# ShuoyiHU/pyqed

Measured on AMD Instinct MI355X. Metric: density-matrix steps/sec (N=128 Lindblad) + 2DES grid-points/sec at 1/2/4/8 GPU, higher is better.
Workload: dtype c128; 1 GPU; lindblad_n128_rk4_fp64 (BASELINE.json configs[1]); N=128, n_c_ops=1, batch_per_gpu=256, global_batch=256, parallelism=replicas x1 (independent density matrices per rank, no collective)

## Files before the change

### pyqed_amd/csrc/cgemm_dma128.hpp

```cpp
#pragma once
#include "cgemm_block.hpp"

namespace qd {

constexpr int cg_herm_ctile(int w, int nj) {
  constexpr unsigned short cols[8] = {0x3210, 0x7654, 0x7610, 0x5432, 0x7432, 0x6510, 0x5410, 0x7632};
  return (cols[w] >> (nj * 4)) & 15;
}
constexpr unsigned cg_herm_mask(int w, bool below) {
  unsigned m = 0;
  for (int mi = 0; mi < 2; ++mi)
    for (int nj = 0; nj < 4; ++nj) {
      const int R = mi == 0 ? (w >> 1) : 7 - (w >> 1), C = cg_herm_ctile(w, nj);
      if (below ? R > C : R < C) m |= 1u << (mi * 4 + nj);
    }
  return m;
}

struct CgAcc3 : CgAcc<128> { d4 p3[8]; };

typedef const __attribute__((address_space(1))) void cg_gvoid;
typedef __attribute__((address_space(3))) void cg_lvoid;

__device__ __forceinline__ const char* cg_uniform(const void* p) {
  const unsigned long long v = reinterpret_cast<unsigned long long>(p);
  const unsigned lo = __builtin_amdgcn_readfirstlane((unsigned)v);
  const unsigned hi = __builtin_amdgcn_readfirstlane((unsigned)(v >> 32));
  return reinterpret_cast<const char*>(((unsigned long long)hi << 32) | lo);
}

constexpr int cg_dma_a_kslot(int lr, int k) { return k ^ lr; }
constexpr int cg_dma_a_slot(int r0, int lr, int k) { return (r0 + lr) * CG_KT + cg_dma_a_kslot(lr, k); }
constexpr bool cg_dma_a_slot_bijective() {
  bool seen[128 * CG_KT] = {};
  for (int row = 0; row < 128; ++row)
    for (int k = 0; k < CG_KT; ++k) {
      const int s = cg_dma_a_slot(row & ~15, row & 15, k);
      if (s < 0 || s >= 128 * CG_KT || seen[s]) return false;
      if (cg_dma_a_kslot(row & 15, cg_dma_a_kslot(row & 15, k)) != k) return false;
      seen[s] = true;
    }
  return true;
}
constexpr bool cg_dma_a_slot_conflict_free() {
  for (int r0 = 0; r0 < 128; r0 += 16)
    for (int k = 0; k < CG_KT; ++k) {
      unsigned cols = 0;
      for (int lr = 0; lr < 16; ++lr) {
        const int s = cg_dma_a_slot(r0, lr, k);
        for (int l2 = 0; l2 < lr; ++l2)
          if (cg_dma_a_slot(r0, l2, k) == s) return false;
        cols |= 1u << (s & 15);
      }
      if (cols != 0xffffu) return false;
    }
  return true;
}
static_assert(cg_dma_a_slot_bijective(), "A-tile image: slots");
static_assert(cg_dma_a_slot_conflict_free(), "A-tile image: fragment read groups");

constexpr int cg_dma_b_slot(int k, int col) { return k * 128 + col; }
constexpr int cg_dma_b_k(int e) { return e >> 7; }
constexpr int cg_dma_b_col(int e) { return e & 127; }
constexpr bool cg_dma_b_slot_bijective() {
  bool seen[128 * CG_KT] = {};
  for (int k = 0; k < CG_KT; ++k)
    for (int col = 0; col < 128; ++col) {
      const int s = cg_dma_b_slot(k, col);
      if (s < 0 || s >= 128 * CG_KT || seen[s]) return false;
      if (cg_dma_b_k(s) != k || cg_dma_b_col(s) != col) return false;
      seen[s] = true;
    }
  return true;
}
static_assert(cg_dma_b_slot_bijective(), "B-tile image: slots");

struct CgDmaStage {
  const CgSeg* segs;
  int tps, lda, ldb;
  unsigned offA, offB;
  int wbase;
  __device__ __forceinline__ CgDmaStage(const CgSeg* s, int tps_, int lda_, int ldb_) : segs(s), tps(tps_), lda(lda_), ldb(ldb_) {
    int tid = threadIdx.x;
    asm volatile("" : "+v"(tid));
    const int row = tid >> 4;
    offA = (unsigned)(row * lda + cg_dma_a_kslot(row & 15, tid & 15)) * (unsigned)sizeof(c128);
    offB = (unsigned)(cg_dma_b_k(tid) * ldb + cg_dma_b_col(tid)) * (unsigned)sizeof(c128);
    wbase = __builtin_amdgcn_readfirstlane(tid & ~63);
  }
  __device__ __forceinline__ void issue(int t, CgLds<128>& L, int buf) const {
    const CgSeg sg = segs[t / tps];
    issue_at(sg.A, sg.B, (t % tps) * CG_KT, L, buf);
  }
  __device__ __forceinline__ void issue_at(const c128* A, const c128* B, int kt, CgLds<128>& L, int buf) const {
    const char* ga = cg_uniform(A + kt);
    const char* gb = cg_uniform(B + (size_t)kt * ldb);
#pragma unroll
    for (int q = 0; q < 4; ++q) {
      __builtin_amdgcn_global_load_lds((cg_gvoid*)(ga + (size_t)q * 32 * lda * sizeof(c128) + offA),
                                       (cg_lvoid*)(&L.a[buf][wbase + CG_WG * q]), 16, 0, 0);
      __builtin_amdgcn_global_load_lds((cg_gvoid*)(gb + (size_t)q * 4 * ldb * sizeof(c128) + offB),
                                       (cg_lvoid*)(&L.b[buf][wbase + CG_WG * q]), 16, 0, 0);
    }
  }
  __device__ __forceinline__ void piece(const char* ga, const char* gb, int i, CgLds<128>& L, int buf) const {
    const int q = i & 3;
    if (i >= 4)
      __builtin_amdgcn_global_load_lds((cg_gvoid*)(gb + (size_t)q * 4 * ldb * sizeof(c128) + offB),
                                       (cg_lvoid*)(&L.b[buf][wbase + CG_WG * q]), 16, 0, 0);
    else
      __builtin_amdgcn_global_load_lds((cg_gvoid*)(ga + (size_t)q * 32 * lda * sizeof(c128) + offA),
                                       (cg_lvoid*)(&L.a[buf][wbase + CG_WG * q]), 16, 0, 0);
  }
  __device__ __forceinline__ void issue_b_at(const c128* B, int kt, CgLds<128>& L, int buf) const {
    const char* gb = cg_uniform(B + (size_t)kt * ldb);
#pragma unroll
    for (int q = 0; q < 4; ++q)
      __builtin_amdgcn_global_load_lds((cg_gvoid*)(gb + (size_t)q * 4 * ldb * sizeof(c128) + offB),
                                       (cg_lvoid*)(&L.b[buf][wbase + CG_WG * q]), 16, 0, 0);
  }
};

struct CgNoHook {
  __device__ __forceinline__ void operator()(int) const {}
};

constexpr int CG_STAGE_PER = 2;
struct CgDmaStageHook {
  const CgDmaStage& st;
  CgLds<128>& L;
  const char* ga;
  const char* gb;
  int buf;
  __device__ __forceinline__ void operator()(int p) const {
    static_assert(4 % CG_STAGE_PER == 0, "a point's pieces belong to one half");
    if (p * CG_STAGE_PER >= 8) return;
    if (p * CG_STAGE_PER < 4 ? !ga : !gb) return;
#pragma unroll
    for (int i = p * CG_STAGE_PER; i < (p + 1) * CG_STAGE_PER; ++i) st.piece(ga, gb, i, L, buf);
  }
};

#ifdef QD_PHASE_TIMING
#define CG_KSTAMP_PARAM , unsigned long long (&tk)[6], int tko
#define CG_KSTAMP_ARG(a, o) , a, o
#define CG_KSTAMP_TOP unsigned long long ks0_ = clock64(), ks1_ = ks0_;
#define CG_KSTAMP_END                  \
  cg_sched_fence();                    \
  const unsigned long long ks2_ = clock64(); \
  cg_sched_fence();
#define CG_KSTAMP_BAR                              \
  {                                                \
    const unsigned long long ks3_ = clock64();     \
    tk[tko] += ks1_ - ks0_;                        \
    tk[tko + 1] += ks2_ - ks1_;                    \
    tk[tko + 2] += ks3_ - ks2_;                    \
    ks0_ = ks3_;                                   \
  }
template <class H>
struct CgStampHook {
  const H& h;
  unsigned long long& at;
  __device__ __forceinline__ void operator()(int p) const {
    h(p);
    if (p == 0) {
      cg_sched_fence();
      at = clock64();
      cg_sched_fence();
    }
  }
};
#define CG_KSTAMP_HOOK(h) CgStampHook<decltype(h)>{h, ks1_}
#else
#define CG_KSTAMP_PARAM
#define CG_KSTAMP_ARG(a, o)
#define CG_KSTAMP_TOP
#define CG_KSTAMP_END
#define CG_KSTAMP_BAR
#define CG_KSTAMP_HOOK(h) h
#endif

template <unsigned SK, int Q0, int Q1, class Hook = CgNoHook>
__device__ __forceinline__ void cg_dma_ksteps(const CgLds<128>& L, int buf, CgAcc3& acc, const int (&r0)[2],
                                              const int (&c0)[4], const Hook& hook = Hook()) {
  constexpr int BT = 128, MW = 2, NW = 4;
  constexpr unsigned LIVE = 0xffu & ~SK;
  const int lane = threadIdx.x & 63;
  const int lr = lane & 15, lk = lane >> 4;
#pragma unroll
  for (int q = Q0; q < Q1; ++q) {
    const int kk = 4 * q;
    c128 a[MW];
    double sa[MW];
#pragma unroll
    for (int mi = 0; mi < MW; ++mi) {
      a[mi] = L.a[buf][cg_dma_a_slot(r0[mi], lr, kk + lk)];
      if ((LIVE >> (mi * 4)) & 15u) sa[mi] = a[mi].re + a[mi].im;
    }
#pragma unroll
    for (int h = 0; h < NW; h += 2) {
      c128 b[2];
      double sb[2];
#pragma unroll
      for (int j = 0; j < 2; ++j) {
        const int nj = h + j;
        if (((LIVE >> nj) | (LIVE >> (4 + nj))) & 1u) {
          b[j] = L.b[buf][cg_dma_b_slot(kk + lk, c0[nj] + lr)];
          sb[j] = b[j].re + b[j].im;
        }
      }
      hook(2 * q + h / 2);
#pragma unroll
      for (int mi = 0; mi < MW; ++mi)
#pragma unroll
        for (int j = 0; j < 2; ++j) {
          const int nj = h + j;
          if (SK & (1u << (mi * 4 + nj))) continue;
          acc.re[mi][nj] = __builtin_amdgcn_mfma_f64_16x16x4f64(a[mi].re, b[j].re, acc.re[mi][nj], 0, 0, 0);
        }
#pragma unroll
      for (int mi = 0; mi < MW; ++mi)
#pragma unroll
        for (int j = 0; j < 2; ++j) {
          const int nj = h + j;
          if (SK & (1u << (mi * 4 + nj))) continue;
          acc.im[mi][nj] = __builtin_amdgcn_mfma_f64_16x16x4f64(a[mi].im, b[j].im, acc.im[mi][nj], 0, 0, 0);
          acc.p3[mi * 4 + nj] = __builtin_amdgcn_mfma_f64_16x16x4f64(sa[mi], sb[j], acc.p3[mi * 4 + nj], 0, 0, 0);
        }
    }
  }
}

__device__ __forceinline__ void cg_dma_scale(CgAcc3& acc, unsigned M, double S) {
#pragma unroll
  for (int mi = 0; mi < 2; ++mi)
#pragma unroll
    for (int nj = 0; nj < 4; ++nj)
      if (M & (1u << (mi * 4 + nj))) {
        acc.re[mi][nj] *= S;
        acc.im[mi][nj] *= S;
        acc.p3[mi * 4 + nj] *= S;
      }
}

__device__ __forceinline__ void cg_dma_zero(CgAcc3& acc) {
#pragma unroll
  for (int mi = 0; mi < 2; ++mi)
#pragma unroll
    for (int nj = 0; nj < 4; ++nj) {
      acc.re[mi][nj] = d4{0.0, 0.0, 0.0, 0.0};
      acc.im[mi][nj] = d4{0.0, 0.0, 0.0, 0.0};
      acc.p3[mi * 4 + nj] = d4{0.0, 0.0, 0.0, 0.0};
    }
}

__device__ __forceinline__ void cg_dma_finalise(CgAcc3& acc) {
#pragma unroll
  for (int mi = 0; mi < 2; ++mi)
#pragma unroll
    for (int nj = 0; nj < 4; ++nj) {
      const d4 p1 = acc.re[mi][nj], p2 = acc.im[mi][nj];
      acc.re[mi][nj] = p1 - p2;
      acc.im[mi][nj] = (acc.p3[mi * 4 + nj] - p1) - p2;
      asm volatile("" : "+v"(acc.re[mi][nj]), "+v"(acc.im[mi][nj]));
    }
}

__device__ __forceinline__ void cg_dma_block_gemm_stream(const c128* A, const c128* B, const c128* nA, const c128* nB,
                                                         bool first, int K, int lda, int ldb, CgLds<128>& L,
                                                         CgAcc3& acc) {
  constexpr int MW = CgCfg<128>::MW, NW = CgCfg<128>::NW, WC = CgCfg<128>::WC, NQ = CG_KT / 4;
  const int wave = __builtin_amdgcn_readfirstlane(threadIdx.x >> 6);
  const int wr0 = (wave / WC) * (MW * 16), wc0 = (wave % WC) * (NW * 16);
  const int r0[2] = {wr0, wr0 + 16}, c0[4] = {wc0, wc0 + 16, wc0 + 32, wc0 + 48};
  cg_dma_zero(acc);
  const int T = K / CG_KT;
  const CgDmaStage st(nullptr, T, lda, ldb);
  if (first) {
    st.issue_at(A, B, 0, L, 0);
    __syncthreads();
  }
  for (int t = 0; t < T; ++t) {
    if (t + 1 < T) st.issue_at(A, B, (t + 1) * CG_KT, L, (t + 1) & 1);
    else st.issue_at(nA, nB, 0, L, 0);
    cg_sched_fence();
    cg_dma_ksteps<0u, 0, NQ>(L, t & 1, acc, r0, c0);
    __syncthreads();
  }
  cg_dma_finalise(acc);
}

template <int W, unsigned SK>
__device__ __forceinline__ void cg_dma_herm_x_range(int t0, int t1, int T, const CgDmaStage& st, CgLds<128>& L,
                                                    CgAcc3& acc) {
  constexpr int NQ = CG_KT / 4, R0 = 16 * (W >> 1), R1 = 16 * (7 - (W >> 1));
  const int r0[2] = {R0, R1};
  const int c0[4] = {16 * cg_herm_ctile(W, 0), 16 * cg_herm_ctile(W, 1), 16 * cg_herm_ctile(W, 2),
                     16 * cg_herm_ctile(W, 3)};
  for (int t = t0; t < t1; ++t) {
    if (t + 1 < T) st.issue(t + 1, L, (t + 1) & 1);
    cg_sched_fence();
    cg_dma_ksteps<SK, 0, NQ>(L, t & 1, acc, r0, c0);
    __syncthreads();
  }
}

__device__ __forceinline__ void cg_dma_herm_x_gemm(const CgSeg* segs, int nseg, int K, int lda, int ldb, CgLds<128>& L,
                                                   CgAcc3& acc, bool pre = false) {
  const int wave = __builtin_amdgcn_readfirstlane(threadIdx.x >> 6);
  cg_dma_zero(acc);
  const int tps = K / CG_KT, T = nseg * tps;
  const CgDmaStage st(segs, tps, lda, ldb);
  if (!pre) {
    st.issue(0, L, 0);
    __syncthreads();
  }
  auto run = [&](auto wc) {
    constexpr int W = decltype(wc)::value;
    cg_dma_herm_x_range<W, 0u>(0, tps, T, st, L, acc);
    cg_dma_scale(acc, cg_herm_mask(W, false), 0.5);
    cg_dma_herm_x_range<W, cg_herm_mask(W, true)>(tps, T, T, st, L, acc);
    cg_dma_scale(acc, cg_herm_mask(W, false), 2.0);
  };
#define QD_HT(w) \
  case w: run(std::integral_constant<int, w>{}); break;
  switch (wave) {
    QD_HT(0) QD_HT(1) QD_HT(2) QD_HT(3) QD_HT(4) QD_HT(5) QD_HT(6) default: QD_HT(7)
  }
#undef QD_HT
  cg_dma_finalise(acc);
}

template <unsigned M>
__device__ __forceinline__ void cg_dma_finalise_live(CgAcc3& acc) {
#pragma unroll
  for (int mi = 0; mi < 2; ++mi)
#pragma unroll
    for (int nj = 0; nj < 4; ++nj) {
      if (!(M & (1u << (mi * 4 + nj)))) continue;
      const d4 p1 = acc.re[mi][nj], p2 = acc.im[mi][nj];
      acc.re[mi][nj] = p1 - p2;
      acc.im[mi][nj] = (acc.p3[mi * 4 + nj] - p1) - p2;
      asm volatile("" : "+v"(acc.re[mi][nj]), "+v"(acc.im[mi][nj]));
    }
}


enum CgStart { CG_START_COLD, CG_START_TILE0, CG_START_TWO };
__device__ __forceinline__ void cg_dma_block_gemm_stream_h(const c128* A, const c128* B, const c128* nA, const c128* nB,
                                                           CgStart start, int K, int lda, int ldb, CgLds<128>& L,
                                                           CgAcc3& acc CG_KSTAMP_PARAM) {
  constexpr int MW = CgCfg<128>::MW, NW = CgCfg<128>::NW, WC = CgCfg<128>::WC, NQ = CG_KT / 4;
  const int wave = __builtin_amdgcn_readfirstlane(threadIdx.x >> 6);
  const int wr0 = (wave / WC) * (MW * 16), wc0 = (wave % WC) * (NW * 16);
  const int r0[2] = {wr0, wr0 + 16}, c0[4] = {wc0, wc0 + 16, wc0 + 32, wc0 + 48};
  cg_dma_zero(acc);
  const int T = K / CG_KT;
  const CgDmaStage st(nullptr, T, lda, ldb);
  if (start == CG_START_COLD) {
    st.issue_at(A, B, 0, L, 0);
    __syncthreads();
  }
  CG_KSTAMP_TOP
  for (int t = 0; t < T; ++t) {
    const bool more = t + 1 < T;
    const char* ga = more ? cg_uniform(A + (t + 1) * CG_KT) : nA ? cg_uniform(nA) : nullptr;
    const char* gb = cg_uniform(more ? B + (size_t)(t + 1) * CG_KT * ldb : nB);
    if (start == CG_START_TWO && t == 0) gb = nullptr;
    const CgDmaStageHook hook{st, L, ga, gb, more ? (t + 1) & 1 : 0};
    cg_sched_fence();
    cg_dma_ksteps<0u, 0, NQ>(L, t & 1, acc, r0, c0, CG_KSTAMP_HOOK(hook));
    CG_KSTAMP_END
    asm volatile("s_waitcnt vmcnt(0)" ::: "memory");
    __syncthreads();
    CG_KSTAMP_BAR
  }
  cg_dma_finalise(acc);
}

__device__ __forceinline__ void cg_dma_a_tile_write(const CgAcc3& acc, int mi, int nj, int row0 , int lane,
                                                    CgLds<128>& L, int buf) {
#pragma unroll
  for (int e = 0; e < 4; ++e)
    L.a[buf][cg_dma_a_slot(row0, (lane >> 4) + 4 * e, lane & 15)] = cmk(acc.re[mi][nj][e], acc.im[mi][nj][e]);
}

template <int W>
__device__ __forceinline__ void cg_dma_herm_d_gemm_h(const CgSeg* segs, const c128* nA, int nseg, int K, int lda,
                                                     int ldb, CgLds<128>& L, CgAcc3& acc, bool two CG_KSTAMP_PARAM) {
  constexpr unsigned SK = cg_herm_mask(W, true);
  constexpr int NQ = CG_KT / 4, R0 = 16 * (W >> 1), R1 = 16 * (7 - (W >> 1));
  const int r0[2] = {R0, R1};
  const int c0[4] = {16 * cg_herm_ctile(W, 0), 16 * cg_herm_ctile(W, 1), 16 * cg_herm_ctile(W, 2),
                     16 * cg_herm_ctile(W, 3)};
  cg_dma_zero(acc);
  const int tps = K / CG_KT, T = nseg * tps;
  const CgDmaStage st(segs, tps, lda, ldb);
  int t = 0;
  CG_KSTAMP_TOP
  if (two) {
    cg_sched_fence();
    const CgNoHook none;
    cg_dma_ksteps<SK, 0, NQ>(L, 0, acc, r0, c0, CG_KSTAMP_HOOK(none));
    CG_KSTAMP_END
    asm volatile("s_waitcnt vmcnt(0)" ::: "memory");
    __syncthreads();
    CG_KSTAMP_BAR
    t = 1;
  }
  for (; t < T; ++t) {
    const char *ga = nullptr, *gb = nullptr;
    if (t + 1 == T) {
      if (nA) ga = cg_uniform(nA);
    } else {
      const CgSeg sg = segs[(t + 1) / tps];
      const int kt = ((t + 1) % tps) * CG_KT;
      ga = cg_uniform(sg.A + kt);
      gb = cg_uniform(sg.B + (size_t)kt * ldb);
    }
    const CgDmaStageHook hook{st, L, ga, gb, (t + 1) & 1};
    cg_sched_fence();
    cg_dma_ksteps<SK, 0, NQ>(L, t & 1, acc, r0, c0, CG_KSTAMP_HOOK(hook));
    CG_KSTAMP_END
    asm volatile("s_waitcnt vmcnt(0)" ::: "memory");
    __syncthreads();
    CG_KSTAMP_BAR
  }
}

}
```

### pyqed_amd/csrc/glf_eig_jump.hip

```cpp
#include "glf_eig_jump_kernel.hpp"

#include <algorithm>

using namespace qd;

namespace {

__global__ void eig_jump_prep_kernel(const c128* W, const c128* Wi, const c128* Et, int ne, c128* Wdh, c128* Widh,
                                     c128* eT) {
  constexpr int Np = JUMP_NP;
  constexpr size_t NN = (size_t)Np * Np;
  for (size_t e = blockIdx.x * (size_t)blockDim.x + threadIdx.x; e < NN; e += (size_t)gridDim.x * blockDim.x) {
    const int i = (int)(e / Np), j = (int)(e % Np);
    const size_t t = (size_t)j * Np + i;
    Wdh[t] = cscale(cconj(W[e]), 0.5);
    Widh[t] = cscale(cconj(Wi[e]), 0.5);
    for (int m = 0; m < ne; ++m) eT[m * NN + t] = Et[m * NN + e];
  }
}

}

extern "C" int qd_lindblad_rk4_eig_jump(const qd_c128* mu, const qd_c128* At, const qd_c128* W, const qd_c128* Winv,
                                        qd_c128* rho, int B, int N, double dt, int nsteps, const qd_c128* Et, int ne,
                                        qd_c128* obs, void* stream) {
  QD_CHECK_ARG(mu && At && W && Winv && rho, "qd_lindblad_rk4_eig_jump: mu, At, W, Winv and rho must be non-null");
  QD_CHECK_ARG(N > 64 && N <= JUMP_NP, "qd_lindblad_rk4_eig_jump: N=%d outside (64, 128]", N);
  QD_CHECK_ARG(B >= 1 && nsteps >= 0 && ne >= 0, "qd_lindblad_rk4_eig_jump: bad sizes B=%d nsteps=%d ne=%d", B, nsteps,
               ne);
  QD_CHECK_ARG(ne == 0 || (Et && obs), "qd_lindblad_rk4_eig_jump: Et/obs null but ne=%d", ne);
  hipStream_t st = (hipStream_t)stream;
  WsScope wss_(st);
  constexpr int Np = JUMP_NP;
  constexpr size_t NN = (size_t)Np * Np;
  int rc;
  void* wops = nullptr;
  if ((rc = workspace(WS_LINDBLAD_OPS, (size_t)(2 + ne) * NN * sizeof(c128), &wops, st))) return rc;
  c128* Wdh = (c128*)wops;
  c128* Widh = Wdh + NN;
  c128* eT = Widh + NN;
  const bool pad = Np != N;
  const size_t per = 2 * NN;
  void* wst = nullptr;
  if ((rc = workspace(WS_LINDBLAD, ((size_t)B * per + (pad ? (size_t)B * NN : 0)) * sizeof(c128), &wst, st))) return rc;
  c128* scratch = (c128*)wst;
  c128* rho_p = pad ? scratch + (size_t)B * per : (c128*)rho;
  hipLaunchKernelGGL(eig_jump_prep_kernel, dim3((int)(NN / 256)), dim3(256), 0, st, (const c128*)W, (const c128*)Winv,
                     (const c128*)Et, ne, Wdh, Widh, eT);
  QD_HIP(hipGetLastError());
  if (pad && (rc = glf_pad((const c128*)rho, rho_p, B, N, Np, st))) return rc;
  LindbladJumpParams p{};
  p.At = (const c128*)At;
  p.W = (const c128*)W;
  p.Wi = (const c128*)Winv;
  p.Wdh = Wdh;
  p.Widh = Widh;
  p.mu = (const c128*)mu;
  p.eT = eT;
  p.rho = rho_p;
  p.ws = scratch;
  p.obs = (c128*)obs;
  p.ne = ne;
  p.nsteps = nsteps;
  p.dt = dt;
  p.tbuf = nullptr;
#ifdef QD_PHASE_TIMING
  QD_HIP(hipMalloc(&p.tbuf, (size_t)B * QD_TSTRIDE * sizeof(unsigned long long)));
  QD_HIP(hipMemsetAsync(p.tbuf, 0, (size_t)B * QD_TSTRIDE * sizeof(unsigned long long), st));
#endif
  note_path("glf_eig_jump");
  hipLaunchKernelGGL(lindblad_eig_jump_kernel, dim3(B), dim3(CG_WG), 0, st, p);
  QD_HIP(hipGetLastError());
  if (pad && (rc = glf_unpad(rho_p, (c128*)rho, B, N, Np, st))) return rc;
#ifdef QD_PHASE_TIMING
  {
    std::vector<unsigned long long> t((size_t)B * QD_TSTRIDE);
    QD_HIP(hipStreamSynchronize(st));
    QD_HIP(hipMemcpy(t.data(), p.tbuf, t.size() * sizeof(unsigned long long), hipMemcpyDeviceToHost));
    (void)hipFree(p.tbuf);
    int dev = 0, khz = 100000;
    (void)hipGetDevice(&dev);
    (void)hipDeviceGetAttribute(&khz, hipDeviceAttributeWallClockRate, dev);
    const char* names[6] = {"basis-changes", nullptr, "gemm", "update", "obs", "lds-pass"};
    std::fprintf(stderr, "[qd phase timing] eig_jump N=%d B=%d nsteps=%d, us per step (basis-changes: per call; mean "
                 "over workgroups):", N, B, nsteps);
    for (int q = 0; q < 6; ++q) {
      if (!names[q]) continue;
      double s = 0;
      for (int b = 0; b < B; ++b) s += (double)t[(size_t)b * QD_TSTRIDE + q];
      std::fprintf(stderr, " %s %.2f", names[q], s / B / (khz * 1e-3) / (q == 0 ? 1 : std::max(1, nsteps)));
    }
    double cyc = 0, wt = 0;
    for (int b = 0; b < B; ++b) {
      cyc += (double)t[(size_t)b * QD_TSTRIDE + QD_TCLK];
      wt += (double)t[(size_t)b * QD_TSTRIDE + QD_TWALL];
    }
    std::fprintf(stderr, " | shader clock %.0f MHz\n", wt > 0 ? cyc / (wt / (khz * 1e3)) / 1e6 : 0.0);
  }
#endif
  return QD_OK;
}
```

### pyqed_amd/csrc/glf_eig_jump_kernel.hpp

```cpp
#pragma once
#include "glf_herm_k.hpp"

namespace qd {

struct LindbladJumpParams {
  const c128* At;
  const c128* W;
  const c128* Wi;
  const c128* Wdh;
  const c128* Widh;
  const c128* mu;
  const c128* eT;
  c128* rho;
  c128* ws;
  c128* obs;
  int ne, nsteps;
  double dt;
  unsigned long long* tbuf;
};

namespace {

constexpr int JUMP_NP = 128;
constexpr int JUMP_NPRE = 3;

template <int W>
__device__ __forceinline__ void jump_r_loads(const c128* r, int Np, int lane, c128 (&rq)[8][4]) {
  const unsigned vu = (unsigned)((lane >> 4) * Np + (lane & 15)) * (unsigned)sizeof(c128);
#pragma unroll
  for (int mi = 0; mi < 2; ++mi)
#pragma unroll
    for (int nj = 0; nj < 4; ++nj) {
      const int R = mi == 0 ? (W >> 1) : 7 - (W >> 1), C = cg_herm_ctile(W, nj);
#pragma unroll
      for (int e = 0; e < 4; ++e) {
        const unsigned su = (unsigned)((16 * R + 4 * e) * Np) * (unsigned)sizeof(c128);
        rq[mi * 4 + nj][e] = *reinterpret_cast<const c128*>(reinterpret_cast<const char*>(r + 16 * C) + (vu + su));
      }
    }
}
template <int W>
__device__ __forceinline__ void jump_mu_reads(const c128* muS, int lane, c128 (&mj)[4], c128 (&mi_)[2][4]) {
#pragma unroll
  for (int nj = 0; nj < 4; ++nj) mj[nj] = muS[16 * cg_herm_ctile(W, nj) + (lane & 15)];
#pragma unroll
  for (int mi = 0; mi < 2; ++mi)
#pragma unroll
    for (int e = 0; e < 4; ++e) mi_[mi][e] = muS[16 * (mi == 0 ? (W >> 1) : 7 - (W >> 1)) + (lane >> 4) + 4 * e];
}
__device__ __forceinline__ void jump_init_mr(CgAcc3& acc, c128 (&rq)[8][4], const c128 (&mj)[4],
                                             const c128 (&mi_)[2][4]) {
#pragma unroll
  for (int mi = 0; mi < 2; ++mi)
#pragma unroll
    for (int nj = 0; nj < 4; ++nj) {
#pragma unroll
      for (int e = 0; e < 4; ++e) {
        const c128 a = mi_[mi][e], b = mj[nj], x = rq[mi * 4 + nj][e];
        const double mre = 0.5 * (a.re * b.re + a.im * b.im), mim = 0.5 * (a.im * b.re - a.re * b.im);
        rq[mi * 4 + nj][e] = cmk(mre * x.re - mim * x.im, mre * x.im + mim * x.re);
      }
#pragma unroll
      for (int e = 0; e < 4; ++e) asm volatile("" : "+v"(rq[mi * 4 + nj][e].re), "+v"(rq[mi * 4 + nj][e].im));
    }
  cg_sched_fence();
#pragma unroll
  for (int mi = 0; mi < 2; ++mi)
#pragma unroll
    for (int nj = 0; nj < 4; ++nj)
#pragma unroll
      for (int e = 0; e < 4; ++e) {
        const c128 t = rq[mi * 4 + nj][e];
        acc.re[mi][nj][e] = t.re;
        acc.im[mi][nj][e] = 0.0;
        acc.p3[mi * 4 + nj][e] = t.re + t.im;
      }
}

template <int W>
__device__ __forceinline__ void jump_gemm(const c128* A, const c128* B, const c128* r, bool mr, const c128* muS, int Np,
                                          int lane, CgLds<128>& L, CgAcc3& acc) {
  constexpr int NQ = CG_KT / 4, R0 = 16 * (W >> 1), R1 = 16 * (7 - (W >> 1));
  const int r0[2] = {R0, R1};
  const int c0[4] = {16 * cg_herm_ctile(W, 0), 16 * cg_herm_ctile(W, 1), 16 * cg_herm_ctile(W, 2),
                     16 * cg_herm_ctile(W, 3)};
  const int T = Np / CG_KT;
  const CgDmaStage st(nullptr, T, Np, Np);
  if (mr) {
    c128 rq[8][4], mj[4], mi_[2][4];
    jump_r_loads<W>(r, Np, lane, rq);
    jump_mu_reads<W>(muS, lane, mj, mi_);
    asm volatile("s_waitcnt lgkmcnt(0)" ::: "memory");
    cg_sched_fence();
    st.issue_at(A, B, 0, L, 0);
    cg_sched_fence();
    jump_init_mr(acc, rq, mj, mi_);
  } else {
    st.issue_at(A, B, 0, L, 0);
    cg_dma_zero(acc);
  }
  __syncthreads();
  for (int t = 0; t < T; ++t) {
    const bool more = t + 1 < T;
    const char* ga = more ? cg_uniform(A + (t + 1) * CG_KT) : nullptr;
    const char* gb = more ? cg_uniform(B + (size_t)(t + 1) * CG_KT * Np) : nullptr;
    const CgDmaStageHook hook{st, L, ga, gb, (t + 1) & 1};
    cg_sched_fence();
    cg_dma_ksteps<0u, 0, NQ>(L, t & 1, acc, r0, c0, hook);
    asm volatile("s_waitcnt vmcnt(0)" ::: "memory");
    __syncthreads();
  }
  cg_dma_finalise(acc);
}

template <int W, int NPRE>
__device__ __forceinline__ void jump_update(const CgAcc<128>& A, const c128* KL, int lane, c128 (&q)[8][4],
                                            const c128* base, c128* rn, int Np, double a, double hc) {
  const int lr = lane >> 4, lc = lane & 15;
  const unsigned vu = (unsigned)(lr * Np + lc) * (unsigned)sizeof(c128);
  const unsigned vm = (unsigned)(lc * Np + lr) * (unsigned)sizeof(c128);
  int n = 0;
#pragma unroll
  for (int mi = 0; mi < 2; ++mi)
#pragma unroll
    for (int nj = 0; nj < 4; ++nj) {
      const int R = mi == 0 ? (W >> 1) : 7 - (W >> 1), C = cg_herm_ctile(W, nj);
      if (R > C) continue;
      if (n >= 1) {
        cg_sched_fence();
        herm_k_rho_loads<W>(base, Np, lane, q, n - 1 + NPRE, n + NPRE);
        cg_sched_fence();
      }
      ++n;
      c128 m[4];
#pragma unroll
      for (int r = 0; r < 4; ++r) {
        const int ra = lr + 4 * r;
        if (R < C) m[r] = KL[HermKL::tile(R, C) + HermKL::slot(ra, lc)];
        else m[r] = KL[HermKL::DIAG0 + R * 128 + HermKL::dslot(ra, lc)];
      }
#pragma unroll
      for (int r = 0; r < 4; ++r) {
        const c128 x = cmk(A.re[mi][nj][r], A.im[mi][nj][r]);
        const int ra = lr + 4 * r;
        const c128 k = cadd(x, R == C && ra == lc ? cconj(x) : m[r]);
        c128 v = cadd(cscale(q[mi * 4 + nj][r], a), cscale(k, hc));
        if (R == C && ra == lc) v.im = 0.0;
        const unsigned su = (unsigned)((16 * R + 4 * r) * Np) * (unsigned)sizeof(c128);
        const unsigned sm = (unsigned)(16 * C * Np) * (unsigned)sizeof(c128);
        char* u = reinterpret_cast<char*>(rn + 16 * C) + (vu + su);
        char* t = reinterpret_cast<char*>(rn + 16 * R + 4 * r) + (vm + sm);
        if (R < C || ra <= lc) *reinterpret_cast<c128*>(u) = v;
        if (R < C || ra < lc) *reinterpret_cast<c128*>(t) = cconj(v);
      }
    }
}

template <int W>
__device__ __forceinline__ void jump_store_y(const CgAcc<128>& A, c128* Y, int Np, int lane) {
  const unsigned vu = (unsigned)((lane >> 4) * Np + (lane & 15)) * (unsigned)sizeof(c128);
#pragma unroll
  for (int mi = 0; mi < 2; ++mi)
#pragma unroll
    for (int nj = 0; nj < 4; ++nj) {
      const int R = mi == 0 ? (W >> 1) : 7 - (W >> 1), C = cg_herm_ctile(W, nj);
#pragma unroll
      for (int e = 0; e < 4; ++e) {
        const unsigned su = (unsigned)((16 * R + 4 * e) * Np) * (unsigned)sizeof(c128);
        *reinterpret_cast<c128*>(reinterpret_cast<char*>(Y + 16 * C) + (vu + su)) = cmk(A.re[mi][nj][e], A.im[mi][nj][e]);
      }
    }
}

__global__ __launch_bounds__(CG_WG) void lindblad_eig_jump_kernel(LindbladJumpParams p) {
  constexpr int BT = JUMP_NP;
  constexpr size_t NN = (size_t)JUMP_NP * JUMP_NP;
  int Np = JUMP_NP;
  asm volatile("" : "+s"(Np));
  __shared__ CgLds<BT> L;
  __shared__ c128 sred[CG_WG / 64];
  __shared__ c128 muS[JUMP_NP];

  const int b = blockIdx.x;
  c128* rho = p.rho + (size_t)b * NN;
  c128* ws = p.ws + (size_t)b * 2 * NN;
  c128* rbuf1 = ws + NN;
  c128* obs = p.obs ? p.obs + (size_t)b * (p.nsteps + 1) * p.ne : nullptr;
  if (threadIdx.x < JUMP_NP) muS[threadIdx.x] = p.mu[threadIdx.x];
  __syncthreads();

  CgAcc3 A;
  QD_TIMING_DECL
#ifdef QD_PHASE_TIMING
  unsigned long long txf = 0;
#endif

  const int nit = 4 * p.nsteps + 4;
  for (int it = 0; it < nit; ++it) {
    const bool xf = it < 2 || it >= nit - 2, ypass = it == 0 || it == nit - 2;
    const int stage = (it - 2) & 3;
    const c128* r = (xf || stage == 0) ? rho : ((stage - 1) & 1) ? rbuf1 : ws;
    c128* rn = (xf || stage == 3) ? rho : (stage & 1) ? rbuf1 : ws;
    const c128* oa = it == 0 ? p.Wi : it == nit - 2 ? p.W : xf ? ws : p.At;
    const c128* ob = it == 1 ? p.Widh : it == nit - 1 ? p.Wdh : r;
    double dts = p.dt;
    asm volatile("" : "+s"(dts));
    const double hc = wave_uniform(xf ? 1.0 : glf_horner_coef(dts, stage)), ab = wave_uniform(xf ? 0.0 : 1.0);
#ifdef QD_PHASE_TIMING
    unsigned long long tkeep[6] = {tacc[0], tacc[1], tacc[2], tacc[3], tacc[4], tacc[5]};
#endif
    {
      static_assert(HermKL::SIZE * sizeof(c128) <= sizeof(CgLds<BT>), "LDS k image");
      c128* KL = reinterpret_cast<c128*>(&L);
      const int wave = __builtin_amdgcn_readfirstlane(threadIdx.x >> 6);
      auto pass = [&](auto wc) {
        constexpr int W = decltype(wc)::value;
        {
          int tid = threadIdx.x;
          asm volatile("" : "+v"(tid));
          jump_gemm<W>(oa, ob, r, !xf, muS, Np, tid & 63, L, A);
        }
        QD_TMARK(2);
        int tid = threadIdx.x;
        asm volatile("" : "+v"(tid));
        const int lane = tid & 63;
        int Npe = Np;
        asm volatile("" : "+s"(Npe));
        if (ypass) {
          jump_store_y<W>(A, ws, Npe, lane);
          return;
        }
        c128 q[8][4];
        herm_k_publish<W>(A, KL, lane);
        cg_sched_fence();
        herm_k_rho_loads<W>(rho, Npe, lane, q, 0, JUMP_NPRE);
        __syncthreads();
        QD_TMARK(5);
        jump_update<W, JUMP_NPRE>(A, KL, lane, q, rho, rn, Npe, ab, hc);
      };
#define QD_JW(w) \
  case w: pass(std::integral_constant<int, w>{}); break;
      switch (wave) { QD_JW(0) QD_JW(1) QD_JW(2) QD_JW(3) QD_JW(4) QD_JW(5) QD_JW(6) default: QD_JW(7) }
#undef QD_JW
      __syncthreads();
    }
    QD_TMARK(3);
#ifdef QD_PHASE_TIMING
    if (xf)
      for (int q = 0; q < 6; ++q) {
        txf += tacc[q] - tkeep[q];
        tacc[q] = tkeep[q];
      }
#endif
    if (p.ne > 0 && (it == 1 || (!xf && stage == 3))) {
      wg_observables_batch(rho, p.eT, p.ne, NN, obs + (size_t)((it - 1) / 4) * p.ne, sred);
      QD_TMARK(4);
    }
  }
#ifdef QD_PHASE_TIMING
  tacc[0] += txf;
#endif
  QD_TIMING_FLUSH
}

}
}
```

Measured before the change: 988,700 density-matrix steps/s.

## Exploit Hermitian structure in jump-operator GEMM and fuse stage tail via LDS

```diff
diff --git a/pyqed_amd/csrc/cgemm_dma128.hpp b/pyqed_amd/csrc/cgemm_dma128.hpp
--- a/pyqed_amd/csrc/cgemm_dma128.hpp
+++ b/pyqed_amd/csrc/cgemm_dma128.hpp
@@ -428,4 +428,93 @@
   }
 }
 
-}
+constexpr unsigned cg_xh_row(unsigned m, int mi) { return (m >> (mi * 4)) & 15u; }
+constexpr unsigned cg_xh_col(unsigned m, int nj) { return ((m >> nj) | (m >> (4 + nj))) & 1u; }
+constexpr int cg_xh_diag_row(unsigned dg, int nj) { return (dg >> nj) & 1u ? 0 : (dg >> (4 + nj)) & 1u ? 1 : -1; }
+
+template <unsigned FS, unsigned SW, unsigned DG, int Q0, int Q1, class Hook = CgNoHook>
+__device__ __forceinline__ void cg_dma_ksteps_xh(const CgLds<128>& L, int buf, CgAcc3& acc, const int (&r0)[2],
+                                                 const int (&c0)[4], const Hook& hook = Hook()) {
+  static_assert((SW & ~FS) == 0u && (DG & ~FS) == 0u && (DG & SW) == 0u, "SW and DG are disjoint subsets of FS");
+  constexpr int MW = 2, NW = 4;
+  const int lane = threadIdx.x & 63;
+  const int lr = lane & 15, lk = lane >> 4;
+#pragma unroll
+  for (int q = Q0; q < Q1; ++q) {
+    const int kk = 4 * q;
+    c128 a[MW], br[MW];
+    double sa[MW], sbr[MW], dbr[MW];
+#pragma unroll
+    for (int mi = 0; mi < MW; ++mi) {
+      if (cg_xh_row(FS, mi)) {
+        a[mi] = L.a[buf][cg_dma_a_slot(r0[mi], lr, kk + lk)];
+        sa[mi] = a[mi].re + a[mi].im;
+      }
+      if (cg_xh_row(SW, mi)) {
+        br[mi] = L.b[buf][cg_dma_b_slot(kk + lk, r0[mi] + lr)];
+        dbr[mi] = br[mi].re - br[mi].im;
+        if (cg_xh_row(DG, mi)) sbr[mi] = br[mi].re + br[mi].im;
+      }
+    }
+#pragma unroll
+    for (int h = 0; h < NW; h += 2) {
+      c128 b[2], ac[2];
+      double sb[2], dac[2];
+#pragma unroll
+      for (int j = 0; j < 2; ++j) {
+        const int nj = h + j, dm = cg_xh_diag_row(DG, nj);
+        if (cg_xh_col(FS, nj)) {
+          if (dm >= 0 && cg_xh_row(SW, dm)) {
+            b[j] = br[dm];
+            sb[j] = sbr[dm];
+          } else {
+            b[j] = L.b[buf][cg_dma_b_slot(kk + lk, c0[nj] + lr)];
+            sb[j] = b[j].re + b[j].im;
+          }
+        }
+        if (cg_xh_col(SW, nj)) {
+          if (dm >= 0) ac[j] = a[dm];
+          else ac[j] = L.a[buf][cg_dma_a_slot(c0[nj], lr, kk + lk)];
+          dac[j] = ac[j].re - ac[j].im;
+        }
+      }
+      hook(2 * q + h / 2);
+#pragma unroll
+      for (int mi = 0; mi < MW; ++mi)
+#pragma unroll
+        for (int j = 0; j < 2; ++j) {
+          const int nj = h + j;
+          if (!(FS & (1u << (mi * 4 + nj)))) continue;
+          acc.re[mi][nj] = __builtin_amdgcn_mfma_f64_16x16x4f64(a[mi].re, b[j].re, acc.re[mi][nj], 0, 0, 0);
+        }
+#pragma unroll
+      for (int mi = 0; mi < MW; ++mi)
+#pragma unroll
+        for (int j = 0; j < 2; ++j) {
+          const int nj = h + j;
+          if (!(FS & (1u << (mi * 4 + nj)))) continue;
+          acc.im[mi][nj] = __builtin_amdgcn_mfma_f64_16x16x4f64(a[mi].im, b[j].im, acc.im[mi][nj], 0, 0, 0);
+          acc.p3[mi * 4 + nj] = __builtin_amdgcn_mfma_f64_16x16x4f64(sa[mi], sb[j], acc.p3[mi * 4 + nj], 0, 0, 0);
+        }
+#pragma unroll
+      for (int mi = 0; mi < MW; ++mi)
+#pragma unroll
+        for (int j = 0; j < 2; ++j) {
+          const int nj = h + j;
+          if (!(SW & (1u << (mi * 4 + nj)))) continue;
+          acc.re[mi][nj] = __builtin_amdgcn_mfma_f64_16x16x4f64(br[mi].re, ac[j].re, acc.re[mi][nj], 0, 0, 0);
+        }
+#pragma unroll
+      for (int mi = 0; mi < MW; ++mi)
+#pragma unroll
+        for (int j = 0; j < 2; ++j) {
+          const int nj = h + j;
+          if (!(SW & (1u << (mi * 4 + nj)))) continue;
+          acc.im[mi][nj] = __builtin_amdgcn_mfma_f64_16x16x4f64(br[mi].im, ac[j].im, acc.im[mi][nj], 0, 0, 0);
+          acc.p3[mi * 4 + nj] = __builtin_amdgcn_mfma_f64_16x16x4f64(dbr[mi], dac[j], acc.p3[mi * 4 + nj], 0, 0, 0);
+        }
+    }
+  }
+}
+
+}
diff --git a/pyqed_amd/csrc/glf_eig_jump.hip b/pyqed_amd/csrc/glf_eig_jump.hip
--- a/pyqed_amd/csrc/glf_eig_jump.hip
+++ b/pyqed_amd/csrc/glf_eig_jump.hip
@@ -81,7 +81,7 @@
     int dev = 0, khz = 100000;
     (void)hipGetDevice(&dev);
     (void)hipDeviceGetAttribute(&khz, hipDeviceAttributeWallClockRate, dev);
-    const char* names[6] = {"basis-changes", nullptr, "gemm", "update", "obs", "lds-pass"};
+    const char* names[6] = {"basis-changes", nullptr, "gemm", "tail", "obs", nullptr};
     std::fprintf(stderr, "[qd phase timing] eig_jump N=%d B=%d nsteps=%d, us per step (basis-changes: per call; mean "
                  "over workgroups):", N, B, nsteps);
     for (int q = 0; q < 6; ++q) {
diff --git a/pyqed_amd/csrc/glf_eig_jump_kernel.hpp b/pyqed_amd/csrc/glf_eig_jump_kernel.hpp
--- a/pyqed_amd/csrc/glf_eig_jump_kernel.hpp
+++ b/pyqed_amd/csrc/glf_eig_jump_kernel.hpp
@@ -22,154 +22,267 @@
 namespace {
 
 constexpr int JUMP_NP = 128;
-constexpr int JUMP_NPRE = 3;
-
-template <int W>
-__device__ __forceinline__ void jump_r_loads(const c128* r, int Np, int lane, c128 (&rq)[8][4]) {
-  const unsigned vu = (unsigned)((lane >> 4) * Np + (lane & 15)) * (unsigned)sizeof(c128);
-#pragma unroll
-  for (int mi = 0; mi < 2; ++mi)
-#pragma unroll
-    for (int nj = 0; nj < 4; ++nj) {
-      const int R = mi == 0 ? (W >> 1) : 7 - (W >> 1), C = cg_herm_ctile(W, nj);
-#pragma unroll
-      for (int e = 0; e < 4; ++e) {
-        const unsigned su = (unsigned)((16 * R + 4 * e) * Np) * (unsigned)sizeof(c128);
-        rq[mi * 4 + nj][e] = *reinterpret_cast<const c128*>(reinterpret_cast<const char*>(r + 16 * C) + (vu + su));
-      }
-    }
-}
-template <int W>
-__device__ __forceinline__ void jump_mu_reads(const c128* muS, int lane, c128 (&mj)[4], c128 (&mi_)[2][4]) {
-#pragma unroll
-  for (int nj = 0; nj < 4; ++nj) mj[nj] = muS[16 * cg_herm_ctile(W, nj) + (lane & 15)];
-#pragma unroll
-  for (int mi = 0; mi < 2; ++mi)
-#pragma unroll
-    for (int e = 0; e < 4; ++e) mi_[mi][e] = muS[16 * (mi == 0 ? (W >> 1) : 7 - (W >> 1)) + (lane >> 4) + 4 * e];
-}
-__device__ __forceinline__ void jump_init_mr(CgAcc3& acc, c128 (&rq)[8][4], const c128 (&mj)[4],
-                                             const c128 (&mi_)[2][4]) {
-#pragma unroll
-  for (int mi = 0; mi < 2; ++mi)
-#pragma unroll
-    for (int nj = 0; nj < 4; ++nj) {
-#pragma unroll
-      for (int e = 0; e < 4; ++e) {
-        const c128 a = mi_[mi][e], b = mj[nj], x = rq[mi * 4 + nj][e];
-        const double mre = 0.5 * (a.re * b.re + a.im * b.im), mim = 0.5 * (a.im * b.re - a.re * b.im);
-        rq[mi * 4 + nj][e] = cmk(mre * x.re - mim * x.im, mre * x.im + mim * x.re);
-      }
-#pragma unroll
-      for (int e = 0; e < 4; ++e) asm volatile("" : "+v"(rq[mi * 4 + nj][e].re), "+v"(rq[mi * 4 + nj][e].im));
-    }
-  cg_sched_fence();
-#pragma unroll
-  for (int mi = 0; mi < 2; ++mi)
-#pragma unroll
-    for (int nj = 0; nj < 4; ++nj)
-#pragma unroll
-      for (int e = 0; e < 4; ++e) {
-        const c128 t = rq[mi * 4 + nj][e];
-        acc.re[mi][nj][e] = t.re;
-        acc.im[mi][nj][e] = 0.0;
-        acc.p3[mi * 4 + nj][e] = t.re + t.im;
-      }
-}
-
-template <int W>
-__device__ __forceinline__ void jump_gemm(const c128* A, const c128* B, const c128* r, bool mr, const c128* muS, int Np,
-                                          int lane, CgLds<128>& L, CgAcc3& acc) {
-  constexpr int NQ = CG_KT / 4, R0 = 16 * (W >> 1), R1 = 16 * (7 - (W >> 1));
-  const int r0[2] = {R0, R1};
-  const int c0[4] = {16 * cg_herm_ctile(W, 0), 16 * cg_herm_ctile(W, 1), 16 * cg_herm_ctile(W, 2),
-                     16 * cg_herm_ctile(W, 3)};
+
+constexpr int jump_ctile(int w, int nj) {
+  constexpr unsigned short cols[8] = {0x3210, 0x7654, 0x4321, 0x7650, 0x7432, 0x6510, 0x7632, 0x5410};
+  return (cols[w] >> (nj * 4)) & 15;
+}
+constexpr int jump_rtile(int w, int mi) { return mi == 0 ? (w >> 1) : 7 - (w >> 1); }
+enum JumpTiles { JUMP_UPPER, JUMP_ABOVE, JUMP_DIAG };
+constexpr unsigned jump_mask(int w, JumpTiles kind) {
+  unsigned m = 0;
+  for (int mi = 0; mi < 2; ++mi)
+    for (int nj = 0; nj < 4; ++nj) {
+      const int R = jump_rtile(w, mi), C = jump_ctile(w, nj);
+      if (kind == JUMP_UPPER ? R <= C : kind == JUMP_ABOVE ? R < C : R == C) m |= 1u << (mi * 4 + nj);
+    }
+  return m;
+}
+constexpr bool jump_tiles_partition() {
+  int n[8][8] = {};
+  for (int w = 0; w < 8; ++w)
+    for (int mi = 0; mi < 2; ++mi)
+      for (int nj = 0; nj < 4; ++nj) ++n[jump_rtile(w, mi)][jump_ctile(w, nj)];
+  for (int R = 0; R < 8; ++R)
+    for (int C = 0; C < 8; ++C)
+      if (n[R][C] != 1) return false;
+  return true;
+}
+constexpr bool jump_tiles_balanced() {
+  for (int s = 0; s < 4; ++s) {
+    int d = 0, o = 0;
+    for (int w = s; w < 8; w += 4)
+      for (int t = 0; t < 8; ++t) {
+        d += (jump_mask(w, JUMP_DIAG) >> t) & 1u;
+        o += (jump_mask(w, JUMP_ABOVE) >> t) & 1u;
+      }
+    if (d != 2 || o != 7) return false;
+  }
+  return true;
+}
+static_assert(jump_tiles_partition(), "jump_ctile: a partition of the 64 tiles");
+static_assert(jump_tiles_balanced(), "jump_ctile: 2 diagonal + 7 off-diagonal tiles per SIMD");
+
+constexpr bool jump_rn_lds_upper(int R, int C, int ra, int lc) { return R < 2 && (R < C || ra <= lc); }
+constexpr bool jump_rn_lds_mirror(int R, int C, int ra, int lc) { return C < 2 && (R < C || ra < lc); }
+constexpr bool jump_rn_lds_one_to_one() {
+  unsigned char n[2][CG_KT * JUMP_NP] = {};
+  for (int w = 0; w < 8; ++w)
+    for (int mi = 0; mi < 2; ++mi)
+      for (int nj = 0; nj < 4; ++nj) {
+        const int R = jump_rtile(w, mi), C = jump_ctile(w, nj);
+        if (R > C) continue;
+        if ((R < 2 || C < 2) && !(w < 4 && mi == 0)) return false;
+        for (int lane = 0; lane < 64; ++lane)
+          for (int e = 0; e < 4; ++e) {
+            const int ra = (lane >> 4) + 4 * e, lc = lane & 15;
+            if (jump_rn_lds_upper(R, C, ra, lc)) ++n[R][cg_dma_b_slot(ra, 16 * C + lc)];
+            if (jump_rn_lds_mirror(R, C, ra, lc)) ++n[C][cg_dma_b_slot(lc, 16 * R + ra)];
+          }
+      }
+  for (int t = 0; t < 2; ++t)
+    for (int s = 0; s < CG_KT * JUMP_NP; ++s)
+      if (n[t][s] != 1) return false;
+  return true;
+}
+static_assert(jump_rn_lds_one_to_one(), "rows 0 .. 31 of rn onto L.b[0], L.b[1]: one writer per slot");
+
+constexpr int jump_patch_slot(int ra, int cc) { return ra * 16 + (cc ^ ra); }
+static_assert(8 * 256 <= JUMP_NP * CG_SA, "the eight patches fit L.a[1]");
+
+template <int W, bool FULL>
+__device__ __forceinline__ void jump_gemm(const c128* A, const c128* B, const c128* nA, CgStart start, int Np,
+                                          CgLds<128>& L, CgAcc3& acc) {
+  constexpr int NQ = CG_KT / 4;
+  constexpr unsigned FS = jump_mask(W, JUMP_UPPER), SW = jump_mask(W, JUMP_ABOVE), DG = jump_mask(W, JUMP_DIAG);
+  const int r0[2] = {16 * jump_rtile(W, 0), 16 * jump_rtile(W, 1)};
+  const int c0[4] = {16 * jump_ctile(W, 0), 16 * jump_ctile(W, 1), 16 * jump_ctile(W, 2), 16 * jump_ctile(W, 3)};
   const int T = Np / CG_KT;
   const CgDmaStage st(nullptr, T, Np, Np);
-  if (mr) {
-    c128 rq[8][4], mj[4], mi_[2][4];
-    jump_r_loads<W>(r, Np, lane, rq);
-    jump_mu_reads<W>(muS, lane, mj, mi_);
-    asm volatile("s_waitcnt lgkmcnt(0)" ::: "memory");
-    cg_sched_fence();
+  if constexpr (FULL) cg_dma_zero(acc);
+  if (start == CG_START_COLD) {
     st.issue_at(A, B, 0, L, 0);
-    cg_sched_fence();
-    jump_init_mr(acc, rq, mj, mi_);
-  } else {
-    st.issue_at(A, B, 0, L, 0);
-    cg_dma_zero(acc);
+    __syncthreads();
   }
-  __syncthreads();
   for (int t = 0; t < T; ++t) {
     const bool more = t + 1 < T;
-    const char* ga = more ? cg_uniform(A + (t + 1) * CG_KT) : nullptr;
+    const char* ga = more ? cg_uniform(A + (t + 1) * CG_KT) : nA ? cg_uniform(nA) : nullptr;
     const char* gb = more ? cg_uniform(B + (size_t)(t + 1) * CG_KT * Np) : nullptr;
-    const CgDmaStageHook hook{st, L, ga, gb, (t + 1) & 1};
+    if (start == CG_START_TWO && t == 0) gb = nullptr;
+    const CgDmaStageHook hook{st, L, ga, gb, more ? (t + 1) & 1 : 0};
     cg_sched_fence();
-    cg_dma_ksteps<0u, 0, NQ>(L, t & 1, acc, r0, c0, hook);
+    if constexpr (FULL) cg_dma_ksteps<0u, 0, NQ>(L, t & 1, acc, r0, c0, hook);
+    else cg_dma_ksteps_xh<FS, SW, DG, 0, NQ>(L, t & 1, acc, r0, c0, hook);
     asm volatile("s_waitcnt vmcnt(0)" ::: "memory");
     __syncthreads();
   }
-  cg_dma_finalise(acc);
-}
-
-template <int W, int NPRE>
-__device__ __forceinline__ void jump_update(const CgAcc<128>& A, const c128* KL, int lane, c128 (&q)[8][4],
-                                            const c128* base, c128* rn, int Np, double a, double hc) {
+}
+
+template <int W>
+__device__ __forceinline__ void jump_tile_loads(const c128* m, int lane, c128 (&q)[8][4]) {
+  const unsigned vu = (unsigned)((lane >> 4) * JUMP_NP + (lane & 15)) * (unsigned)sizeof(c128);
+#pragma unroll
+  for (int mi = 0; mi < 2; ++mi)
+#pragma unroll
+    for (int nj = 0; nj < 4; ++nj) {
+      const int R = jump_rtile(W, mi), C = jump_ctile(W, nj);
+      if (R > C) continue;
+#pragma unroll
+      for (int e = 0; e < 4; ++e) {
+        const unsigned su = (unsigned)((16 * R + 4 * e) * JUMP_NP) * (unsigned)sizeof(c128);
+        q[mi * 4 + nj][e] = *reinterpret_cast<const c128*>(reinterpret_cast<const char*>(m + 16 * C) + (vu + su));
+      }
+    }
+}
+
+template <int W>
+__device__ __forceinline__ void jump_tail(CgAcc3& A, const c128* base, c128* rn, const c128* muS, CgLds<128>& L,
+                                          int lane, double a, double hc, double gn) {
+  constexpr unsigned LIVE = jump_mask(W, JUMP_UPPER);
   const int lr = lane >> 4, lc = lane & 15;
-  const unsigned vu = (unsigned)(lr * Np + lc) * (unsigned)sizeof(c128);
-  const unsigned vm = (unsigned)(lc * Np + lr) * (unsigned)sizeof(c128);
-  int n = 0;
-#pragma unroll
-  for (int mi = 0; mi < 2; ++mi)
-#pragma unroll
-    for (int nj = 0; nj < 4; ++nj) {
-      const int R = mi == 0 ? (W >> 1) : 7 - (W >> 1), C = cg_herm_ctile(W, nj);
+  const unsigned vu = (unsigned)(lr * JUMP_NP + lc) * (unsigned)sizeof(c128);
+  const unsigned vm = (unsigned)(lc * JUMP_NP + lr) * (unsigned)sizeof(c128);
+  c128 q[8][4];
+  cg_dma_finalise_live<LIVE>(A);
+  cg_sched_fence();
+  jump_tile_loads<W>(base, lane, q);
+  c128* P = &L.a[1][256 * W];
+#pragma unroll
+  for (int mi = 0; mi < 2; ++mi)
+#pragma unroll
+    for (int nj = 0; nj < 4; ++nj) {
+      const int R = jump_rtile(W, mi), C = jump_ctile(W, nj);
+      if (R != C) continue;
+#pragma unroll
+      for (int e = 0; e < 4; ++e) P[jump_patch_slot(lr + 4 * e, lc)] = cmk(A.re[mi][nj][e], A.im[mi][nj][e]);
+#pragma unroll
+      for (int e = 0; e < 4; ++e) {
+        const c128 m = P[jump_patch_slot(lc, lr + 4 * e)];
+        A.re[mi][nj][e] += m.re;
+        A.im[mi][nj][e] -= m.im;
+      }
+    }
+#pragma unroll
+  for (int mi = 0; mi < 2; ++mi)
+#pragma unroll
+    for (int nj = 0; nj < 4; ++nj) {
+      const int R = jump_rtile(W, mi), C = jump_ctile(W, nj);
       if (R > C) continue;
-      if (n >= 1) {
-        cg_sched_fence();
-        herm_k_rho_loads<W>(base, Np, lane, q, n - 1 + NPRE, n + NPRE);
-        cg_sched_fence();
-      }
-      ++n;
-      c128 m[4];
-#pragma unroll
-      for (int r = 0; r < 4; ++r) {
-        const int ra = lr + 4 * r;
-        if (R < C) m[r] = KL[HermKL::tile(R, C) + HermKL::slot(ra, lc)];
-        else m[r] = KL[HermKL::DIAG0 + R * 128 + HermKL::dslot(ra, lc)];
-      }
-#pragma unroll
-      for (int r = 0; r < 4; ++r) {
-        const c128 x = cmk(A.re[mi][nj][r], A.im[mi][nj][r]);
-        const int ra = lr + 4 * r;
-        const c128 k = cadd(x, R == C && ra == lc ? cconj(x) : m[r]);
-        c128 v = cadd(cscale(q[mi * 4 + nj][r], a), cscale(k, hc));
+      const c128 mj = muS[16 * C + lc];
+      const double gs = R == C ? 0.5 * gn : gn;
+#pragma unroll
+      for (int e = 0; e < 4; ++e) {
+        const int ra = lr + 4 * e;
+        const c128 k = cmk(A.re[mi][nj][e], A.im[mi][nj][e]);
+        c128 v = cadd(cscale(q[mi * 4 + nj][e], a), cscale(k, hc));
         if (R == C && ra == lc) v.im = 0.0;
-        const unsigned su = (unsigned)((16 * R + 4 * r) * Np) * (unsigned)sizeof(c128);
-        const unsigned sm = (unsigned)(16 * C * Np) * (unsigned)sizeof(c128);
+        const unsigned su = (unsigned)((16 * R + 4 * e) * JUMP_NP) * (unsigned)sizeof(c128);
+        const unsigned sm = (unsigned)(16 * C * JUMP_NP) * (unsigned)sizeof(c128);
         char* u = reinterpret_cast<char*>(rn + 16 * C) + (vu + su);
-        char* t = reinterpret_cast<char*>(rn + 16 * R + 4 * r) + (vm + sm);
+        char* t = reinterpret_cast<char*>(rn + 16 * R + 4 * e) + (vm + sm);
         if (R < C || ra <= lc) *reinterpret_cast<c128*>(u) = v;
         if (R < C || ra < lc) *reinterpret_cast<c128*>(t) = cconj(v);
+        if constexpr (W < 4) {
+          if (R < 2 && jump_rn_lds_upper(R, C, ra, lc)) L.b[R & 1][cg_dma_b_slot(ra, 16 * C + lc)] = v;
+          if (R < 2 && C < 2 && jump_rn_lds_mirror(R, C, ra, lc)) L.b[C & 1][cg_dma_b_slot(lc, 16 * R + ra)] = cconj(v);
+        }
+        const c128 mi_ = muS[16 * R + ra];
+        const double gre = gs * (mi_.re * mj.re + mi_.im * mj.im), gim = gs * (mi_.im * mj.re - mi_.re * mj.im);
+        const double tre = gre * v.re - gim * v.im, tim = gre * v.im + gim * v.re;
+        A.re[mi][nj][e] = tre;
+        A.im[mi][nj][e] = 0.0;
+        A.p3[mi * 4 + nj][e] = tre + tim;
       }
     }
 }
 
 template <int W>
-__device__ __forceinline__ void jump_store_y(const CgAcc<128>& A, c128* Y, int Np, int lane) {
-  const unsigned vu = (unsigned)((lane >> 4) * Np + (lane & 15)) * (unsigned)sizeof(c128);
-#pragma unroll
-  for (int mi = 0; mi < 2; ++mi)
-#pragma unroll
-    for (int nj = 0; nj < 4; ++nj) {
-      const int R = mi == 0 ? (W >> 1) : 7 - (W >> 1), C = cg_herm_ctile(W, nj);
+__device__ __forceinline__ void jump_store_y(const CgAcc<128>& A, c128* Y, int lane) {
+  const unsigned vu = (unsigned)((lane >> 4) * JUMP_NP + (lane & 15)) * (unsigned)sizeof(c128);
+#pragma unroll
+  for (int mi = 0; mi < 2; ++mi)
+#pragma unroll
+    for (int nj = 0; nj < 4; ++nj) {
+      const int R = jump_rtile(W, mi), C = jump_ctile(W, nj);
 #pragma unroll
       for (int e = 0; e < 4; ++e) {
-        const unsigned su = (unsigned)((16 * R + 4 * e) * Np) * (unsigned)sizeof(c128);
+        const unsigned su = (unsigned)((16 * R + 4 * e) * JUMP_NP) * (unsigned)sizeof(c128);
         *reinterpret_cast<c128*>(reinterpret_cast<char*>(Y + 16 * C) + (vu + su)) = cmk(A.re[mi][nj][e], A.im[mi][nj][e]);
       }
     }
+}
+
+struct JumpCall {
+  const c128 *At, *W, *Wi, *Wdh, *Widh, *eT;
+  c128 *rho, *ws, *rbuf1, *obs;
+  int ne, nit;
+  double dt;
+};
+
+#ifdef QD_PHASE_TIMING
+#define JUMP_TIMING_PARAM , const LindbladJumpParams& p, unsigned long long (&tacc)[6], unsigned long long& tlast, unsigned long long& txf
+#define JUMP_TIMING_ARG , p, tacc, tlast, txf
+#else
+#define JUMP_TIMING_PARAM
+#define JUMP_TIMING_ARG
+#endif
+
+template <int W>
+__device__ __forceinline__ void jump_run(const JumpCall o, int Np, CgLds<128>& L, c128* sred, const c128* muS JUMP_TIMING_PARAM) {
+  const int nit = o.nit;
+  CgAcc3 A;
+  for (int it = 0; it < nit; ++it) {
+    const bool xf = it < 2 || it >= nit - 2, ypass = it == 0 || it == nit - 2;
+    const int stage = (it - 2) & 3;
+    const c128* r = (xf || stage == 0) ? o.rho : ((stage - 1) & 1) ? o.rbuf1 : o.ws;
+    c128* rn = (xf || stage == 3) ? o.rho : (stage & 1) ? o.rbuf1 : o.ws;
+    const c128* oa = it == 0 ? o.Wi : it == nit - 2 ? o.W : xf ? o.ws : o.At;
+    const c128* ob = it == 1 ? o.Widh : it == nit - 1 ? o.Wdh : r;
+    const c128* na = (ypass || it == nit - 1) ? nullptr : it + 1 == nit - 2 ? o.W : o.At;
+    const CgStart start = (it == 0 || it == 1 || it == nit - 1) ? CG_START_COLD : CG_START_TWO;
+    double dts = o.dt;
+    asm volatile("" : "+s"(dts));
+    const double hc = wave_uniform(xf ? 1.0 : glf_horner_coef(dts, stage)), ab = wave_uniform(xf ? 0.0 : 1.0);
+    const double gn = wave_uniform(it >= 1 && it + 1 < nit - 2 ? 1.0 : 0.0);
+    const bool watch = o.ne > 0 && (it == 1 || (!xf && stage == 3));
+#ifdef QD_PHASE_TIMING
+    unsigned long long tkeep[6] = {tacc[0], tacc[1], tacc[2], tacc[3], tacc[4], tacc[5]};
+#endif
+    if (ypass) {
+      jump_gemm<W, true>(oa, ob, na, start, Np, L, A);
+      cg_dma_finalise(A);
+      QD_TMARK(2);
+      int tid = threadIdx.x;
+      asm volatile("" : "+v"(tid));
+      jump_store_y<W>(A, o.ws, tid & 63);
+      cg_dma_zero(A);
+    } else {
+      jump_gemm<W, false>(oa, ob, na, start, Np, L, A);
+      QD_TMARK(2);
+      int tid = threadIdx.x;
+      asm volatile("" : "+v"(tid));
+      jump_tail<W>(A, o.rho, rn, muS, L, tid & 63, ab, hc, gn);
+    }
+    if (ypass || watch || it == nit - 1) {
+      __syncthreads();
+    } else {
+      asm volatile("s_waitcnt lgkmcnt(0)" ::: "memory");
+      __builtin_amdgcn_s_barrier();
+      asm volatile("" ::: "memory");
+    }
+    QD_TMARK(3);
+#ifdef QD_PHASE_TIMING
+    if (xf)
+      for (int q = 0; q < 6; ++q) {
+        txf += tacc[q] - tkeep[q];
+        tacc[q] = tkeep[q];
+      }
+#endif
+    if (watch) {
+      wg_observables_batch(o.rho, o.eT, o.ne, JUMP_NP * (size_t)JUMP_NP, o.obs + (size_t)((it - 1) / 4) * o.ne, sred);
+      QD_TMARK(4);
+    }
+  }
 }
 
 __global__ __launch_bounds__(CG_WG) void lindblad_eig_jump_kernel(LindbladJumpParams p) {
@@ -189,74 +302,18 @@
   if (threadIdx.x < JUMP_NP) muS[threadIdx.x] = p.mu[threadIdx.x];
   __syncthreads();
 
-  CgAcc3 A;
   QD_TIMING_DECL
 #ifdef QD_PHASE_TIMING
   unsigned long long txf = 0;
 #endif
 
   const int nit = 4 * p.nsteps + 4;
-  for (int it = 0; it < nit; ++it) {
-    const bool xf = it < 2 || it >= nit - 2, ypass = it == 0 || it == nit - 2;
-    const int stage = (it - 2) & 3;
-    const c128* r = (xf || stage == 0) ? rho : ((stage - 1) & 1) ? rbuf1 : ws;
-    c128* rn = (xf || stage == 3) ? rho : (stage & 1) ? rbuf1 : ws;
-    const c128* oa = it == 0 ? p.Wi : it == nit - 2 ? p.W : xf ? ws : p.At;
-    const c128* ob = it == 1 ? p.Widh : it == nit - 1 ? p.Wdh : r;
-    double dts = p.dt;
-    asm volatile("" : "+s"(dts));
-    const double hc = wave_uniform(xf ? 1.0 : glf_horner_coef(dts, stage)), ab = wave_uniform(xf ? 0.0 : 1.0);
-#ifdef QD_PHASE_TIMING
-    unsigned long long tkeep[6] = {tacc[0], tacc[1], tacc[2], tacc[3], tacc[4], tacc[5]};
-#endif
-    {
-      static_assert(HermKL::SIZE * sizeof(c128) <= sizeof(CgLds<BT>), "LDS k image");
-      c128* KL = reinterpret_cast<c128*>(&L);
-      const int wave = __builtin_amdgcn_readfirstlane(threadIdx.x >> 6);
-      auto pass = [&](auto wc) {
-        constexpr int W = decltype(wc)::value;
-        {
-          int tid = threadIdx.x;
-          asm volatile("" : "+v"(tid));
-          jump_gemm<W>(oa, ob, r, !xf, muS, Np, tid & 63, L, A);
-        }
-        QD_TMARK(2);
-        int tid = threadIdx.x;
-        asm volatile("" : "+v"(tid));
-        const int lane = tid & 63;
-        int Npe = Np;
-        asm volatile("" : "+s"(Npe));
-        if (ypass) {
-          jump_store_y<W>(A, ws, Npe, lane);
-          return;
-        }
-        c128 q[8][4];
-        herm_k_publish<W>(A, KL, lane);
-        cg_sched_fence();
-        herm_k_rho_loads<W>(rho, Npe, lane, q, 0, JUMP_NPRE);
-        __syncthreads();
-        QD_TMARK(5);
-        jump_update<W, JUMP_NPRE>(A, KL, lane, q, rho, rn, Npe, ab, hc);
-      };
+  const JumpCall o{p.At, p.W, p.Wi, p.Wdh, p.Widh, p.eT, rho, ws, rbuf1, obs, p.ne, nit, p.dt};
+  const int wave = __builtin_amdgcn_readfirstlane(threadIdx.x >> 6);
 #define QD_JW(w) \
-  case w: pass(std::integral_constant<int, w>{}); break;
-      switch (wave) { QD_JW(0) QD_JW(1) QD_JW(2) QD_JW(3) QD_JW(4) QD_JW(5) QD_JW(6) default: QD_JW(7) }
+  case w: jump_run<w>(o, Np, L, sred, muS JUMP_TIMING_ARG); break;
+  switch (wave) { QD_JW(0) QD_JW(1) QD_JW(2) QD_JW(3) QD_JW(4) QD_JW(5) QD_JW(6) default: QD_JW(7) }
 #undef QD_JW
-      __syncthreads();
-    }
-    QD_TMARK(3);
-#ifdef QD_PHASE_TIMING
-    if (xf)
-      for (int q = 0; q < 6; ++q) {
-        txf += tacc[q] - tkeep[q];
-        tacc[q] = tkeep[q];
-      }
-#endif
-    if (p.ne > 0 && (it == 1 || (!xf && stage == 3))) {
-      wg_observables_batch(rho, p.eT, p.ne, NN, obs + (size_t)((it - 1) / 4) * p.ne, sred);
-      QD_TMARK(4);
-    }
-  }
 #ifdef QD_PHASE_TIMING
   tacc[0] += txf;
 #endif
```

New measurement: 1.190 million density-matrix steps/s (median of 6 runs). +20.3%, better.
